# michel-aractingi/soloRL

Measured on AMD Instinct MI355X. Metric: env-steps/s (whole node) Solo12 walk, 4096 envs/GPU, higher is better.
Workload: dtype f32

## Files before the change

solorl_amd/csrc/dynamics.hpp:

```cpp
#pragma once
#include <utility>

#include "../../include/solorl_model_data.h"
#include "spatial.hpp"

namespace solo {

constexpr int MAX_CONTACTS = 8;
constexpr int MAX_LIMITS = 4;
constexpr int LIM_SLOT_ROWS = 2;
constexpr int MAX_ROWS = LIM_SLOT_ROWS + 3 * MAX_CONTACTS;
SD int extra_limits(int nlt) { return nlt > LIM_SLOT_ROWS ? nlt - LIM_SLOT_ROWS : 0; }
SD int contact_cap(int nlt) { return MAX_CONTACTS - extra_limits(nlt); }
constexpr int ROW_CORE = 20;
constexpr int NPRIM = 24;
constexpr double LIMIT_WINDOW = 0.0;
constexpr double DISC_EPS2 = 1e-12;
constexpr double DISC_RIM = 0.1;

#if defined(SOLO_WAVE_TIMING) && !defined(SOLO_HOST_SHIM)
constexpr int SOLO_WT_WAVES = 65536, SOLO_WT_FIELDS = 28;
__device__ unsigned long long solo_wave_times[SOLO_WT_WAVES][SOLO_WT_FIELDS];
__shared__ unsigned long long solo_pt_acc[10];
#define SOLO_PT_DECL() long long pt_last_ = 0
// ... 1231 lines not shown
      }
    }
    mask = team_or16(keep);
  }
  const int nl = __builtin_popcount(lbits);
  if (valid && t >= 4 && ((mask >> (t - 4)) & 1)) {
    const int p = t - 4, nlt = nl, nc = __builtin_popcount(mask);
    const int cidx = __builtin_popcount(mask & ((1 << p) - 1));
    const int sn_ = nlt + cidx, sf_ = nlt + nc + 2 * cidx;
    const T lam0 = pp.warm * C.lamp[p];
    const T Z[3] = {T(0), T(0), T(0)};
    static_for<3>([&](auto dc) {
      constexpr int d = decltype(dc)::value;
      const V3<T> u = d == 0 ? mk(T(0), T(0), T(1)) : (d == 1 ? mk(T(1), T(0), T(0)) : mk(T(0), T(1), T(0)));
      park_row(lds, d == 0 ? sn_ : sf_ + (d - 1), SV<T>{cross(bP, u), u}, Z, Z, bP, bdist + pp.slop, d == 0 ? lam0 : T(0), bfric,
               (d == 0 ? 0 : (sn_ | 128)) | (d << 8));
    });
  }
  if (!lead) return;
  C.R0 = R0;
  C.mask = mask; C.nc = __builtin_popcount(mask); C.nlim_total = nl; C.lsel = lbits;
  C.smask = sbits & mask;
  constexpr solorl_link_data B = RB::MD.links[0];
  static_assert(B.com[0] == 0.0 && B.com[1] == 0.0 && B.com[2] == 0.0, "base COM at its origin");
  RBI<T> Ib; SV<T> pb;
  const SV<T> vb{st.w, st.v};
  SOLO_LINK_TERMS_CE(UI, B, R0, mk(T(0), T(0), T(0)), vb, pp.damping, Ib, pb);
  C.Ibase = to_abi(Ib); C.pbase = pb;
}

template <typename T, int ROBOT, typename CH>
SD void team_sum_base(CH ch, int t) {
  SubCtx<T, ROBOT>& C = ch.get();
  constexpr int NA = (int)(sizeof(ABI<T>) / sizeof(T)), NP = (int)(sizeof(SV<T>) / sizeof(T));
  static_assert(NA == 21 && NP == 6, "ABI / SV are plain arrays of T");
  T* ib = reinterpret_cast<T*>(&C.Ibase); T* pb = reinterpret_cast<T*>(&C.pbase);
  const T* il = reinterpret_cast<const T*>(&C.Ileg[0]); const T* pl = reinterpret_cast<const T*>(&C.pleg[0]);
#pragma unroll
  for (int k = 0; k < 2; k++) {
    const int i = t + 16 * k;
    if (i < NA) ib[i] = ib[i] + ((il[i] + il[NA + i]) + (il[2 * NA + i] + il[3 * NA + i]));
    else if (i < NA + NP) { const int j = i - NA; pb[j] = pb[j] + ((pl[j] + pl[NP + j]) + (pl[2 * NP + j] + pl[3 * NP + j])); }
  }
}

template <typename T, int ROBOT, typename LDS, typename CH>
SNI_SCALAR void phase_base_lead(CH ch, const PhysParams<T> pp, const T* lam_prev, unsigned nstride, const LDS lds) {
  SubCtx<T, ROBOT>& C = ch.get();
  using TRW = TeamRows<T, LDS>;
  constexpr int LN = LDS::LANES;
  const int nlt = C.nlim_total, nc = C.nc;
  const ABI<T> Ib = C.Ibase;
  const SV<T> pb = C.pbase;
  const V3<T> bw = C.ps.w, bv = C.ps.v;
  const Sym6<T> Lam = spd_inverse_block(Ib);
  const SV<T> a0 = mul(Lam, pb) * T(-1);
  const T dt = pp.dt;
  V3<T> vdot = a0.l + cross(bw, bv); vdot.z -= pp.gravity;
  SV<T> ub;
  ub.a = mk(clampv(bw.x + dt * a0.a.x, pp.vmax), clampv(bw.y + dt * a0.a.y, pp.vmax), clampv(bw.z + dt * a0.a.z, pp.vmax));
  ub.l = mk(clampv(bv.x + dt * vdot.x, pp.vmax), clampv(bv.y + dt * vdot.y, pp.vmax), clampv(bv.z + dt * vdot.z, pp.vmax));
  if (nlt + 3 * nc == 0) {
    const T Z[3] = {T(0), T(0), T(0)};
    park_row(lds, 0, zero6<T>(), Z, Z, mk(T(0), T(0), T(0)), T(0), T(0), T(0), 0);
  }
  C.ub = ub;
  T* bc = TRW::bc(lds.lane);
#pragma unroll
  for (int i = 0; i < 6; i++)
#pragma unroll
    for (int j = 0; j < 6; j++) bc[i * 6 + j] = Lam.m[i][j];
  bc[36] = ub.a.x; bc[37] = ub.a.y; bc[38] = ub.a.z; bc[39] = ub.l.x; bc[40] = ub.l.y; bc[41] = ub.l.z;
  bc[54] = a0.a.x; bc[55] = a0.a.y; bc[56] = a0.a.z; bc[57] = a0.l.x; bc[58] = a0.l.y; bc[59] = a0.l.z;
  T* hdr = lds.hdr();
  hdr[0] = T(nlt); hdr[LN] = T(nc);
}

template <typename T, int ROBOT, typename LDS, typename CH>
SD void phase_legrates_team(CH ch, const PhysParams<T> pp, const LDS lds, int t) {
  using RB = Robot<ROBOT>;
  using TRW = TeamRows<T, LDS>;
  constexpr int NJ = RB::NJ;
  T* bc = TRW::bc(lds.lane);
  if (t < RB::NQ) {
    SubCtx<T, ROBOT>& C = ch.get();
    const int L = t / NJ, k = t - L * NJ;
    const SV<T> a0{{bc[54], bc[55], bc[56]}, {bc[57], bc[58], bc[59]}};
    const T qdd = C.LR[L].qdd0[k] - dot(C.LR[L].G[k], a0);
    const T v = clampv(C.ps.qd[t] + pp.dt * qdd, pp.vmax);
    C.qds[t] = v;
    bc[42 + L * 3 + k] = v;
  } else if (NJ < 3 && t < 12) {
    if ((t - RB::NQ) < 4) bc[42 + (t - RB::NQ) * 3 + 2] = T(0);
  }
}

template <typename T, typename LDS> SD void team_counts(const LDS& lds, int& nlt, int& nc, int& ncmax, int& anylim) {
  const T* hdr = lds.hdr();
  nlt = (int)hdr[0]; nc = (int)hdr[LDS::LANES];
  int m = (nc + extra_limits(nlt)) | (nlt << 8);
#pragma unroll
  for (int o = 32; o >= 16; o >>= 1) { int v = __shfl_xor(m, o); m = ((v & 255) > (m & 255) ? (v & 255) : (m & 255)) | ((v | m) & ~255); }
  m = __builtin_amdgcn_readfirstlane(m);
  ncmax = m & 255; anylim = m >> 8;
}

template <typename T, int ROBOT, typename LDS>
SNI_SCALAR void phase_finish_team(const PhysParams<T> pp, const LDS lds, int t) {
  using TRW = TeamRows<T, LDS>;
  const int col = lds.lane;
  int nlt, nc, ncmax, anylim;
  team_counts<T, LDS>(lds, nlt, nc, ncmax, anylim);
  const int nrows = nlt + 3 * nc, rfric = nlt + nc;
  T* const lam = TRW::lam(col);
  const T* bc = TRW::bc(col);
  for (int pos = t; pos < TRW::TR; pos += 16)
    if (TRW::row_of(pos, nlt, nc) < 0) lam[pos * 4] = T(0);
  if (t >= nrows) return;
  Sym6<T> Lam;
#pragma unroll
  for (int i = 0; i < 6; i++)
#pragma unroll
    for (int j = 0; j < 6; j++) Lam.m[i][j] = bc[i * 6 + j];
  const SV<T> ub{{bc[36], bc[37], bc[38]}, {bc[39], bc[40], bc[41]}};
  const int r1 = t + 16;
  const bool two = r1 < nrows;
  T c0[ROW_CORE], c1[ROW_CORE];
  lds.load_core(t, c0);
  const int meta0 = (int)lds.A(t, LDS::A_META);
  const T mu0 = lds.A(t, LDS::A_MU);
  int meta1 = 0; T mu1 = T(1);
  if (two) { lds.load_core(r1, c1); meta1 = (int)lds.A(r1, LDS::A_META); mu1 = lds.A(r1, LDS::A_MU); }
  auto emit = [&](int r, const T (&c)[ROW_CORE], int meta, T mu) __attribute__((always_inline)) {
    const int leg = (meta >> 5) & 3;
    const T* ql = bc + 42 + leg * 3;
    SV<T> W; T rhs, dinv;
    finish_row(c, meta, Lam, ub, ql[0], ql[1], ql[2], pp, W, rhs, dinv);
    const bool fr = r >= rfric;
    const T sB = fr ? mu : T(1);
    const T isB = rcp_fast(sB);
    const T sJ = dinv * isB;
    T o[ROW_CORE];
#pragma unroll
    for (int e = 0; e < 9; e++) o[E_J(e)] = c[e] * sJ;
    o[E_B(0)] = W.a.x * sB; o[E_B(1)] = W.a.y * sB; o[E_B(2)] = W.a.z * sB; o[E_B(3)] = W.l.x * sB; o[E_B(4)] = W.l.y * sB; o[E_B(5)] = W.l.z * sB;
    o[E_B(6)] = c[15] * sB; o[E_B(7)] = c[16] * sB; o[E_B(8)] = c[17] * sB;
    o[E_RHS] = rhs * isB;
    o[E_LEG] = T(leg);
    lds.store_core(r, o);
    lds.A(r, LDS::A_LAM) = (fr && pp.cone()) ? rcp_fast(pp.resid_thr * sJ) : pp.resid_thr * sJ;
    lam[TRW::pos_of(r, nlt, nc) * 4] = c[13];
  };
  emit(t, c0, meta0, mu0);
  if (two) emit(r1, c1, meta1, mu1);
}

template <typename T> SD T half_swap(T x) {
  if constexpr (sizeof(T) == 4) return __int_as_float(__builtin_amdgcn_mov_dpp(__float_as_int(x), 0x140, 0xF, 0xF, true));
  else return __shfl_xor(x, 8, 16);
}

template <typename T> SD T team_red8(T x) {
  if constexpr (sizeof(T) == 4) {
    x += __int_as_float(__builtin_amdgcn_mov_dpp(__float_as_int(x), 0xB1, 0xF, 0xF, true));
    x += __int_as_float(__builtin_amdgcn_mov_dpp(__float_as_int(x), 0x4E, 0xF, 0xF, true));
    x += __int_as_float(__builtin_amdgcn_mov_dpp(__float_as_int(x), 0x141, 0xF, 0xF, true));
  } else {
    x += __shfl_xor(x, 1, 16); x += __shfl_xor(x, 2, 16); x += __shfl_xor(x, 4, 16);
  }
  return x;
}

#ifndef SOLO_SETUP_GROUP_F32
#define SOLO_SETUP_GROUP_F32 5
#endif
#ifndef SOLO_SETUP_GROUP_F64
#define SOLO_SETUP_GROUP_F64 1
#endif
template <typename T, typename LDS, int LIM, int NNS, int NFS, bool EXIT, bool PIPE = true, bool CONE = false>
SNI void pgs_team_variant(int iterations_v, const LDS lds, int t) {
  using TRW = TeamRows<T, LDS>;
  const int itv = __builtin_amdgcn_readfirstlane(iterations_v);
  const int iterations = itv & 0xFFFF;
  const bool warm_on = (itv >> 30) & 1;
  constexpr int LN = LDS::LANES, n = LIM + NNS + NFS;
  constexpr int S_N0 = 1, S_F0 = 1 + MAX_CONTACTS / 2;
  static_assert(n >= 1, "empty sweeps are not instantiated");
  struct Ord { static constexpr int slot(int i) { return i < LIM ? 0 : (i < LIM + NNS ? S_N0 + (i - LIM) : S_F0 + (i - LIM - NNS)); } };
  const int col = lds.lane;
  const int h = t & 7, half = t >> 3;
  constexpr int SZ = (int)sizeof(T);
  constexpr int S_LAM = 4 * SZ;
  const int lam_own = (int)TRW::off_lam + col * SZ + half * S_LAM;
  const int nlt = (int)lds.hdr()[0], nc = (int)lds.hdr()[LN];
  const int eU = h;
  const int legU = h < 6 ? -1 : 0;
  const int eV = 6 + (h + 2) % 3, legV = (h + 2) / 3;
  const int eW = h < 2 ? 7 + h : 8, legW = h < 2 ? 3 : -2;
  constexpr unsigned ROWB = (unsigned)LDS::NCH * LN * 16u;
  auto eoff = [&](int e) -> unsigned { return (unsigned)(e / LDS::PER) * (LN * 16u) + (unsigned)(e % LDS::PER) * SZ + (unsigned)col * 16u; };
  using P2 = T __attribute__((ext_vector_type(2)));
  static_assert(LDS::PER % 2 == 0, "a (J', B~) pair lies inside one 16-byte chunk");
  const unsigned kU = eoff(E_J(eU)), kV = eoff(E_J(eV)), kW = eoff(E_J(eW));
  const unsigned kUB = eoff(E_B(eU)), kVB = eoff(E_B(eV)), kWB = eoff(E_B(eW));
  const unsigned kLEG = eoff(E_LEG), kRHS = eoff(E_RHS);
  auto rd = [&](unsigned rb, unsigned k) -> T { return *reinterpret_cast<const T*>(solo_smem + (rb + k)); };
  auto rd2 = [&](unsigned rb, unsigned k) -> P2 { return *reinterpret_cast<const P2*>(solo_smem + (rb + k)); };
  auto fm = [](auto a, auto b, auto c) { return __builtin_elementwise_fma(a, b, c); };
  T J0[n], J1[n], J2[n], B2[n], X2[n], rh[n], cp[n], lm[n], eo[n], ex[n];
  P2 B01[n], X01[n];
  T th[EXIT ? n : 1];
  T thx[(EXIT && CONE && NFS > 0) ? NFS : 1];
  T lmo[NNS > 0 ? NNS : 1];
  P2 a01 = {T(0), T(0)}; T a2 = T(0);
  int rown[n], roth[n];
  T lego[n], legx[n];
  T ju[n], bu[n], jv[n], bv[n], jw[n], bw[n], xu[n], xv[n], xw[n], rhs_[n];
  constexpr int SETUP_GROUP = sizeof(T) == 4 ? SOLO_SETUP_GROUP_F32 : SOLO_SETUP_GROUP_F64;
  static_for<(n + SETUP_GROUP - 1) / SETUP_GROUP>([&](auto gc) {
    constexpr int g0 = decltype(gc)::value * SETUP_GROUP, gn = (n - g0 < SETUP_GROUP ? n - g0 : SETUP_GROUP);
    static_for<gn>([&](auto jc) {
      constexpr int i = g0 + decltype(jc)::value;
      constexpr int k = Ord::slot(i);
      constexpr bool fr = i >= LIM + NNS;
      rown[i] = TRW::row_of(2 * k + half, nlt, nc);
      if constexpr (fr) roth[i] = rown[i] < 0 ? -1 : rown[i] + 1 - 2 * half;
      else roth[i] = TRW::row_of(2 * k + 1 - half, nlt, nc);
      const int ro = rown[i] < 0 ? 0 : rown[i], rx = roth[i] < 0 ? 0 : roth[i];
      const unsigned bo = __umul24((unsigned)ro, ROWB), bx = __umul24((unsigned)rx, ROWB);
      lego[i] = rd(bo, kLEG);
      if constexpr (!fr) legx[i] = rd(bx, kLEG); else legx[i] = T(0);
      { const P2 u = rd2(bo, kU), v = rd2(bo, kV), w = rd2(bo, kW);
        ju[i] = u.x; bu[i] = u.y; jv[i] = v.x; bv[i] = v.y; jw[i] = w.x; bw[i] = w.y; }
      xu[i] = rd(bx, kUB); xv[i] = rd(bx, kVB); xw[i] = rd(bx, kWB);
      rhs_[i] = rd(bo, kRHS);
      if constexpr (EXIT) th[i] = lds.A(ro, LDS::A_LAM);
      lm[i] = *reinterpret_cast<const T*>(solo_smem + lam_own + 2 * k * S_LAM);
    });
#ifndef SOLO_HOST_SHIM
    asm volatile("" ::: "memory");
    static_for<gn>([&](auto jc) {
      constexpr int i = g0 + decltype(jc)::value;
      asm volatile("" : "+v"(ju[i]), "+v"(bu[i]), "+v"(jv[i]), "+v"(bv[i]), "+v"(jw[i]), "+v"(bw[i]), "+v"(xu[i]), "+v"(xv[i]), "+v"(xw[i]),
                        "+v"(rhs_[i]), "+v"(lm[i]), "+v"(lego[i]));
      (void)legx;
      if constexpr (i < LIM + NNS) asm volatile("" : "+v"(legx[i]));
      (void)th;
      if constexpr (EXIT) asm volatile("" : "+v"(th[i]));
    });
#endif
    static_for<gn>([&](auto jc) {
      constexpr int i = g0 + decltype(jc)::value;
      constexpr bool fr = i >= LIM + NNS;
      const int r_own = rown[i], r_oth = roth[i];
      const int lo = r_own < 0 ? -3 : (int)lego[i], lx = fr ? lo : (r_oth < 0 ? -3 : (int)legx[i]);
      const bool uo = r_own >= 0 && (legU == -1 || legU == lo), vo = legV == lo, wo = legW == lo;
      const bool ux = fr ? uo : (r_oth >= 0 && (legU == -1 || legU == lx)), vx = fr ? vo : legV == lx, wx = fr ? wo : legW == lx;
      J0[i] = uo ? ju[i] : T(0); J1[i] = vo ? jv[i] : T(0); J2[i] = wo ? jw[i] : T(0);
      B01[i] = P2{uo ? bu[i] : T(0), vo ? bv[i] : T(0)}; B2[i] = wo ? bw[i] : T(0);
      X01[i] = P2{ux ? xu[i] : T(0), vx ? xv[i] : T(0)}; X2[i] = wx ? xw[i] : T(0);
      rh[i] = r_own >= 0 ? rhs_[i] * T(-0.125) : T(0);
      if constexpr (CONE && fr) {
        cp[i] = T(0);
        (void)thx;
        if constexpr (EXIT) { if (r_own < 0) th[i] = T(0); thx[i - LIM - NNS] = half_swap(th[i]); }
      } else {
        const T c = team_red8(J0[i] * X01[i].x + J1[i] * X01[i].y + J2[i] * X2[i]);
        cp[i] = half ? c : T(0);
      }
      if constexpr (i >= LIM && i < LIM + NNS) lmo[i - LIM] = T(0);
    });
    if (warm_on) {
      static_for<gn>([&](auto jc) {
        constexpr int i = g0 + decltype(jc)::value;
        const T lx_ = half_swap(lm[i]);
        if constexpr (i >= LIM && i < LIM + NNS) lmo[i - LIM] = lx_;
        a01 = fm(X01[i], P2{lx_, lx_}, fm(B01[i], P2{lm[i], lm[i]}, a01)); a2 = fm(X2[i], lx_, fm(B2[i], lm[i], a2));
      });
    }
  });
  static_for<n>([&](auto ic) {
    constexpr int i = decltype(ic)::value, p = (i + n - 1) % n;
    if constexpr (PIPE) {
      eo[i] = team_red8(J0[i] * B01[p].x + J1[i] * B01[p].y + J2[i] * B2[p]);
      ex[i] = team_red8(J0[i] * X01[p].x + J1[i] * X01[p].y + J2[i] * X2[p]);
    } else { eo[i] = T(0); ex[i] = T(0); (void)p; }
  });
  auto jdot = [&](int, T j0, T j1, T j2, T r8) -> T { return team_red8(fm(j0, a01.x, fm(j1, a01.y, fm(j2, a2, r8)))); };
  T dpre = jdot(0, J0[0], J1[0], J2[0], rh[0]);
  T delp = T(0), delxp = T(0);
  T* const hdr = lds.hdr();
#define SOLO_PGS_WRITE_BACK() do { \
    if (h == 0) { \
      static_for<n>([&](auto ic_) { \
        constexpr int i_ = decltype(ic_)::value; \
        *reinterpret_cast<T*>(solo_smem + lam_own + 2 * Ord::slot(i_) * S_LAM) = lm[i_]; \
      }); \
    } \
    if (half == 0) { \
      if (h < 6) hdr[(2 + h) * LN] = a01.x; else lds.y()[(h - 6) * LN] = a01.x; \
      lds.y()[(h + 2) * LN] = a01.y; \
      if (h < 2) lds.y()[(10 + h) * LN] = a2; \
    } } while (0)
  bool fin = false;
#if defined(SOLO_WAVE_TIMING) && defined(SOLO_DEAD_STATS)
  unsigned long long fr_tot = 0, fr_dead = 0;
#endif
  int it_done = 0; (void)it_done;
#pragma unroll 1
  for (int it = 0; it < iterations; it++) {
#if defined(SOLO_WAVE_TIMING) && defined(SOLO_SWEEP_STATS)
    it_done = it + 1;
#endif
    bool viol = false;
    static_for<n>([&](auto ic) {
      constexpr int i = decltype(ic)::value, in = (i + 1) % n;
      constexpr bool fric = i >= LIM + NNS;
      T dnext = T(0), d;
      if constexpr (PIPE) {
        dnext = jdot(in, J0[in], J1[in], J2[in], rh[in]);
        d = fm(ex[i], delxp, fm(eo[i], delp, dpre));
      } else d = jdot(i, J0[i], J1[i], J2[i], rh[i]);
      T hi = T(0);
      if constexpr (fric) {
        constexpr int c = i - LIM - NNS;
        if constexpr (sizeof(T) == 4) hi = __int_as_float(__builtin_amdgcn_mov_dpp(__float_as_int(lm[LIM + (c >> 1)]), 0x150 + 8 * (c & 1), 0xF, 0xF, true));
        else hi = (half == (c & 1)) ? lm[LIM + (c >> 1)] : lmo[c >> 1];
      }
      auto clampb = [&](T x) -> T {
        if constexpr (!fric) return x > T(0) ? x : T(0);
        else if constexpr (sizeof(T) == 4) return __builtin_amdgcn_fmed3f(x, -hi, hi);
        else return x < -hi ? -hi : (x > hi ? hi : x);
      };
#if defined(SOLO_WAVE_TIMING) && defined(SOLO_DEAD_STATS)
      if constexpr (fric) { fr_tot++; if (!__any(hi != T(0) || lm[i] != T(0))) fr_dead++; }
#endif
      T sp = lm[i] - d;
      T sv;
      if constexpr (CONE && fric) {
        const T spx = half_swap(sp);
        const T s2 = fm(sp, sp, fm(spx, spx, T(1e-30)));
        T sc;
        if constexpr (sizeof(T) == 4) {
#ifndef SOLO_HOST_SHIM
          sc = __builtin_amdgcn_fmed3f(hi * __builtin_amdgcn_rsqf(s2), 0.0f, 1.0f);
#else
          sc = hi / sqrt(s2); sc = sc < T(1) ? sc : T(1);
#endif
        } else { sc = hi / sqrt(s2); sc = sc < T(1) ? sc : T(1); }
        sv = sp * sc;
      } else {
        const T dfirst = clampb(sp) - lm[i];
        sp = fm(-cp[i], half_swap(dfirst), sp);
        sv = clampb(sp);
      }
      const T del = sv - lm[i];
      lm[i] = sv;
      const T delx = half_swap(del);
      if constexpr (EXIT) {
        if constexpr (CONE && fric) viol = viol || (fabs(fm(delx, thx[i - LIM - NNS], del * th[i])) > T(1));
        else viol = viol || (fabs(del) > th[i]);
      }
      if constexpr (sizeof(T) != 4 && i >= LIM && i < LIM + NNS) lmo[i - LIM] += delx;
      a01 = fm(X01[i], P2{delx, delx}, fm(B01[i], P2{del, del}, a01));
      a2 = fm(X2[i], delx, fm(B2[i], del, a2));
      dpre = dnext; delp = del; delxp = delx;
    });
    if constexpr (EXIT) {
      const bool quiet = team_or16(viol ? 1 : 0) == 0;
      const bool nw = quiet && !fin;
      if (__any(nw)) {
        if (nw) SOLO_PGS_WRITE_BACK();
        fin = fin || quiet;
        if (__all(fin)) break;
      }
    }
  }
  if constexpr (EXIT) { if (!fin) SOLO_PGS_WRITE_BACK(); }
  else SOLO_PGS_WRITE_BACK();
#if defined(SOLO_WAVE_TIMING) && defined(SOLO_SWEEP_STATS)
  if (threadIdx.x == 0 && blockIdx.x < SOLO_WT_WAVES) { solo_wave_times[blockIdx.x][26] += (unsigned long long)it_done; solo_wave_times[blockIdx.x][27] += 1ull; }
#endif
#if defined(SOLO_WAVE_TIMING) && defined(SOLO_DEAD_STATS)
  if (threadIdx.x == 0 && blockIdx.x < SOLO_WT_WAVES) { solo_wave_times[blockIdx.x][26] += fr_tot; solo_wave_times[blockIdx.x][27] += fr_dead; }
#endif
#undef SOLO_PGS_WRITE_BACK
}

template <typename T, int ROBOT, typename LDS>
SD void phase_pgs_team(int iterations_, bool warm_on, bool early_exit, bool pipe, bool cone, const LDS lds, int t) {
  const int iterations = (iterations_ & 0xFFFF) | (warm_on ? 1 << 30 : 0);
  constexpr int LN = LDS::LANES;
  int nlt, nc, ncmax, anylim;
  team_counts<T, LDS>(lds, nlt, nc, ncmax, anylim);
#if defined(SOLO_WAVE_TIMING)
  if (threadIdx.x == 0 && blockIdx.x < SOLO_WT_WAVES) {
    solo_wave_times[blockIdx.x][4] += (unsigned long long)(ncmax + (ncmax + 1) / 2 + (anylim ? 1 : 0));
    if ((unsigned long long)ncmax > solo_wave_times[blockIdx.x][5]) solo_wave_times[blockIdx.x][5] = (unsigned long long)ncmax;
  }
#endif
#ifndef SOLO_NO_SETPRIO
  if (ncmax >= 7) __builtin_amdgcn_s_setprio(3);
  else if (ncmax >= 5) __builtin_amdgcn_s_setprio(2);
  else if (ncmax >= 3) __builtin_amdgcn_s_setprio(1);
  else __builtin_amdgcn_s_setprio(0);
#endif
#define SOLO_SWEEP_C(N_, F_, C_) do { if (early_exit) { if (anylim) pgs_team_variant<T, LDS, 1, N_, F_, true, true, C_>(iterations, lds, t); \
                                                        else pgs_team_variant<T, LDS, 0, N_, F_, true, true, C_>(iterations, lds, t); } \
                                      else if (pipe) { if (anylim) pgs_team_variant<T, LDS, 1, N_, F_, false, true, C_>(iterations, lds, t); \
                                                       else pgs_team_variant<T, LDS, 0, N_, F_, false, true, C_>(iterations, lds, t); } \
                                      else { if (anylim) pgs_team_variant<T, LDS, 1, N_, F_, false, false, C_>(iterations, lds, t); \
                                             else pgs_team_variant<T, LDS, 0, N_, F_, false, false, C_>(iterations, lds, t); } } while (0)
#define SOLO_SWEEP_L(N_, F_) do { if (cone) SOLO_SWEEP_C(N_, F_, true); else SOLO_SWEEP_C(N_, F_, false); } while (0)
  switch (ncmax) {
    case 0:
      if (anylim) { if (early_exit) pgs_team_variant<T, LDS, 1, 0, 0, true>(iterations, lds, t); else pgs_team_variant<T, LDS, 1, 0, 0, false>(iterations, lds, t); }
      else {
        const int h = t & 7;
        T* const hdr = lds.hdr();
        if ((t >> 3) == 0) {
          if (h < 6) hdr[(2 + h) * LN] = T(0); else lds.y()[(h - 6) * LN] = T(0);
          lds.y()[(h + 2) * LN] = T(0);
          if (h < 2) lds.y()[(10 + h) * LN] = T(0);
        }
      }
      break;
    case 1: SOLO_SWEEP_L(1, 1); break;
    case 2: SOLO_SWEEP_L(1, 2); break;
    case 3: SOLO_SWEEP_L(2, 3); break;
    case 4: SOLO_SWEEP_L(2, 4); break;
    case 5: SOLO_SWEEP_L(3, 5); break;
    case 6: SOLO_SWEEP_L(3, 6); break;
    case 7: SOLO_SWEEP_L(4, 7); break;
    default: SOLO_SWEEP_L(4, 8); break;
  }
#undef SOLO_SWEEP_L
#undef SOLO_SWEEP_C
}

template <typename T, int ROBOT, typename LDS, typename CH>
SNI_SCALAR void phase_integrate_team(CH ch, const PhysParams<T> pp, T* lam_prev, unsigned nstride, const LDS lds, int t, bool valid,
                              bool lead) {
  using RB = Robot<ROBOT>;
  using TRW = TeamRows<T, LDS>;
  constexpr int NJ = RB::NJ, LN = LDS::LANES;
  if (!valid) return;
  SubCtx<T, ROBOT>& C = ch.get();
  const T dt = pp.dt;
  const int mask = C.mask;
  const int nlt = C.nlim_total;
  const T* hdr = lds.hdr();
  const SV<T> w{{hdr[2 * LN], hdr[3 * LN], hdr[4 * LN]}, {hdr[5 * LN], hdr[6 * LN], hdr[7 * LN]}};
  const int tj = t < RB::NQ ? t : 0;
  const int L = tj / NJ, k = tj - L * NJ;
  const T qds = C.qds[tj], yk = lds.y()[(L * 3 + k) * LN], qj = C.ps.q[tj];
  const SV<T> Gk = C.LR[L].G[k];
  const SV<T> ub = C.ub;
  const V3<T> pos = C.ps.pos;
  const T x = C.ps.qx, yq = C.ps.qy, z = C.ps.qz, ww = C.ps.qw;
  const T* lam = TRW::lam(lds.lane);
  const int npos0 = TRW::NPOS0 + extra_limits(nlt);
  T lv[(NPRIM + 15) / 16];
#pragma unroll
  for (int i = 0; i < (NPRIM + 15) / 16; i++) {
    const int p = t + 16 * i;
    const int pp_ = p < NPRIM ? p : 0;
    lv[i] = lam[(npos0 + __builtin_popcount(mask & ((1 << pp_) - 1))) * 4];
    lv[i] = (p < NPRIM && ((mask >> pp_) & 1)) ? lv[i] : T(0);
  }
  const T nvj = clampv(qds + yk - dot(Gk, w), pp.vmax);
  const V3<T> nw = mk(clampv(ub.a.x + w.a.x, pp.vmax), clampv(ub.a.y + w.a.y, pp.vmax), clampv(ub.a.z + w.a.z, pp.vmax));
  const V3<T> nv = mk(clampv(ub.l.x + w.l.x, pp.vmax), clampv(ub.l.y + w.l.y, pp.vmax), clampv(ub.l.z + w.l.z, pp.vmax));
#pragma unroll
  for (int i = 0; i < (NPRIM + 15) / 16; i++) { const int p = t + 16 * i; if (p < NPRIM) C.lamp[p] = lv[i]; }
  if (t < RB::NQ) { C.ps.qd[t] = nvj; C.ps.q[t] = qj + dt * nvj; }
  if (lead) {
    C.ps.w = nw; C.ps.v = nv;
    C.ps.pos = fma3(nv, dt, pos);
    T wn2 = dot(nw, nw), wn = sqrt_fast(wn2), sc, s_, cw;
    sincos_t(T(0.5) * wn * dt, s_, cw);
    if (wn < T(1e-3)) sc = T(0.5) * dt - dt * dt * dt * T(1.0 / 48.0) * wn2; else sc = s_ * rcp_fast(wn);
    T ax = nw.x * sc, ay = nw.y * sc, az = nw.z * sc;
    T nx = cw * x + ax * ww + ay * z - az * yq;
    T ny = cw * yq - ax * z + ay * ww + az * x;
    T nz = cw * z + ax * yq - ay * x + az * ww;
    T nq = cw * ww - ax * x - ay * yq - az * z;
    T inv = rsqrt_fast(nx * nx + ny * ny + nz * nz + nq * nq);
    C.ps.qx = nx * inv; C.ps.qy = ny * inv; C.ps.qz = nz * inv; C.ps.qw = nq * inv;
  }
}

template <typename T, int ROBOT, typename LDS> struct TeamCtx {
  using type = CtxLds<T, ROBOT, TeamRows<T, LDS>::off_ctx>;
  static constexpr size_t bytes = TeamRows<T, LDS>::off_ctx + 4 * sizeof(SubCtx<T, ROBOT>);
};

template <typename T, int ROBOT, typename LDS>
SD int substep_team(const PhysParams<T> pp, T* lam_prev, unsigned nstride, const LDS& lds, int t, bool lead, bool valid) {
  constexpr int LN = LDS::LANES;
  using TRW = TeamRows<T, LDS>;
  using CH = typename TeamCtx<T, ROBOT, LDS>::type;
  const CH ch{lds.lane};
  SOLO_PT_DECL();
  SOLO_PT_BEGIN();
  if (valid && t < Robot<ROBOT>::NQ) {
    SubCtx<T, ROBOT>& C = ch.get();
    T sn, cs;
    sincos_t(C.ps.q[t], sn, cs);
    C.sn[t] = sn; C.cs[t] = cs;
  }
  SOLO_PT(0);
  const bool ui = pp.urdf_inertia();
  if (ui) phase_front_team<T, ROBOT, LDS, CH, true>(ch, pp, lds, t, valid, lead);
  else phase_front_team<T, ROBOT, LDS, CH, false>(ch, pp, lds, t, valid, lead);
  SOLO_PT(1);
#if SOLO_LEG_QUAD
  if (valid) {
    if (ui) phase_leg_rt<T, ROBOT, LDS, CH, true>(ch, pp, lam_prev, nstride, lds, t >> 2, t & 3);
    else phase_leg_rt<T, ROBOT, LDS, CH, false>(ch, pp, lam_prev, nstride, lds, t >> 2, t & 3);
  }
#else
  if (valid && t < 4) {
    if (ui) phase_leg_rt<T, ROBOT, LDS, CH, true>(ch, pp, lam_prev, nstride, lds, t, 0);
    else phase_leg_rt<T, ROBOT, LDS, CH, false>(ch, pp, lam_prev, nstride, lds, t, 0);
  }
#endif
  SOLO_PT(2);
  if (valid) team_sum_base<T, ROBOT, CH>(ch, t);
  SOLO_PT(3);
  if (lead) phase_base_lead<T, ROBOT, LDS, CH>(ch, pp, lam_prev, nstride, lds);
  else if (!valid && t == 0) {
    lds.hdr()[0] = T(0); lds.hdr()[LN] = T(0);
  }
  SOLO_PT(4);
  if (valid) phase_legrates_team<T, ROBOT, LDS, CH>(ch, pp, lds, t);
  SOLO_PT(5);
  phase_finish_team<T, ROBOT, LDS>(pp, lds, t);
  SOLO_PT(6);
  phase_pgs_team<T, ROBOT, LDS>(pp.iterations, pp.warm != T(0), pp.resid_thr >= T(0), pp.pgs_pipe(), pp.cone(), lds, t);
  SOLO_PT(7);
  phase_integrate_team<T, ROBOT, LDS, CH>(ch, pp, lam_prev, nstride, lds, t, valid, lead);
  SOLO_PT(8);
  return lead ? (ch.get().mask | strip_feet_bits(ch.get().smask)) : 0;
}
#endif

template <typename T, int ROBOT, typename LDS>
SD int substep(SubCtx<T, ROBOT>& C, const PhysParams<T> pp, T* lam_prev, unsigned nstride, const LDS& lds) {
  using CH = CtxPriv<T, ROBOT>;
  const CH ch{&C};
  if (pp.urdf_inertia()) {
    phase_detect<T, ROBOT, CH, true>(ch, pp);
    phase_leg<T, ROBOT, 0, LDS, CH, true>(ch, pp, lam_prev, nstride, lds);
    phase_leg<T, ROBOT, 1, LDS, CH, true>(ch, pp, lam_prev, nstride, lds);
    phase_leg<T, ROBOT, 2, LDS, CH, true>(ch, pp, lam_prev, nstride, lds);
    phase_leg<T, ROBOT, 3, LDS, CH, true>(ch, pp, lam_prev, nstride, lds);
  } else {
    phase_detect<T, ROBOT, CH, false>(ch, pp);
    phase_leg<T, ROBOT, 0, LDS, CH, false>(ch, pp, lam_prev, nstride, lds);
    phase_leg<T, ROBOT, 1, LDS, CH, false>(ch, pp, lam_prev, nstride, lds);
    phase_leg<T, ROBOT, 2, LDS, CH, false>(ch, pp, lam_prev, nstride, lds);
    phase_leg<T, ROBOT, 3, LDS, CH, false>(ch, pp, lam_prev, nstride, lds);
  }
  phase_base<T, ROBOT, LDS, CH>(ch, pp, lam_prev, nstride, lds);
  if (pp.cone()) phase_pgs<T, ROBOT, LDS, CH, true>(ch, pp.iterations, pp.resid_thr, lds);
  else phase_pgs<T, ROBOT, LDS, CH>(ch, pp.iterations, pp.resid_thr, lds);
  phase_integrate<T, ROBOT, LDS, CH>(ch, pp, lam_prev, nstride, lds);
  return C.mask | strip_feet_bits(C.smask);
}

}
```

solorl_amd/devcode.py:

```python
import os
import re
import subprocess
import tempfile

LLVM = os.environ.get("ROCM_LLVM_BIN", "/opt/rocm/lib/llvm/bin")


MAGIC = b"__CLANG_OFFLOAD_BUNDLE__"


def _code_objects(lib_path, workdir):
    fat = os.path.join(workdir, "fat.bin")
    subprocess.check_call([os.path.join(LLVM, "llvm-objcopy"), "--dump-section", ".hip_fatbin=" + fat, lib_path, os.path.join(workdir, "x.so")])
    blob = open(fat, "rb").read()
    starts = [m.start() for m in re.finditer(re.escape(MAGIC), blob)]
    out = []
    for k, a in enumerate(starts):
        part = os.path.join(workdir, "fat%d.bin" % k)
        open(part, "wb").write(blob[a:starts[k + 1] if k + 1 < len(starts) else len(blob)])
        co = os.path.join(workdir, "dev%d.co" % k)
        subprocess.check_call([os.path.join(LLVM, "clang-offload-bundler"), "--unbundle", "--type=o", "--input=" + part,
                               "--targets=hipv4-amdgcn-amd-amdhsa--gfx950", "--output=" + co])
        if os.path.getsize(co) > 0:
            out.append(co)
    return out


def disassemble(lib_path):
    out, seen = [], {}
    with tempfile.TemporaryDirectory() as d:
        for co in _code_objects(lib_path, d):
            for line in subprocess.check_output([os.path.join(LLVM, "llvm-objdump"), "-d", co], text=True).splitlines():
                m = re.match(r"^([0-9a-f]+) <([^>]+)>:", line)
                if m:
                    k = seen.get(m.group(2), 0)
                    seen[m.group(2)] = k + 1
                    if k:
                        line = "%s <%s.dup%d>:" % (m.group(1), m.group(2), k)
                out.append(line)
    return "\n".join(out)


def kernel_static_lds(lib_path):
    with tempfile.TemporaryDirectory() as d:
        notes = "\n".join(subprocess.check_output([os.path.join(LLVM, "llvm-readelf"), "--notes", co], text=True) for co in _code_objects(lib_path, d))
    out, size = {}, None
    for line in notes.splitlines():
        m = re.search(r"\.group_segment_fixed_size:\s*(\d+)", line)
        if m:
            size = int(m.group(1))
        m = re.search(r"^\s*\.name:\s*(\S+)", line)
        if m and size is not None:
            out[m.group(1)] = size
            size = None
    return out


def kernel_resources(lib_path):
    with tempfile.TemporaryDirectory() as d:
        notes = "\n".join(subprocess.check_output([os.path.join(LLVM, "llvm-readelf"), "--notes", co], text=True) for co in _code_objects(lib_path, d))
    out, cur, col = {}, None, None
    for line in notes.splitlines():
        m = re.match(r"^(\s*-?\s*)\.([a-z_]+):\s*(\S*)\s*$", line)
        if not m:
            continue
        if m.group(1).strip() == "-" and m.group(2) == "agpr_count":
            cur, col = {}, len(m.group(1))
        if cur is None or len(m.group(1)) != col:
            continue
        if m.group(2) == "name":
            out[m.group(3)] = cur
        elif m.group(3).isdigit():
            cur[m.group(2)] = int(m.group(3))
    return out


def function_stats(lib_path):
    out, cur = {}, None
    for line in disassemble(lib_path).splitlines():
        m = re.match(r"^[0-9a-f]+ <([^>]+)>:", line)
        if m:
            cur = out.setdefault(m.group(1), dict(insts=0, scratch=0, flat=0, **{"global": 0})) if ".dup" not in m.group(1) else None
            continue
        if cur is None or "\t" not in line:
            continue
        op = line.split("\t")[1].strip().split(" ")[0] if len(line.split("\t")) > 1 else ""
        if not op:
            continue
        cur["insts"] += 1
        if op.startswith("scratch_"): cur["scratch"] += 1
        elif op.startswith("flat_"): cur["flat"] += 1
        elif op.startswith("global_"): cur["global"] += 1
    return out


def loop_stats(lib_path, name_filter):
    funcs, cur = {}, None
    for line in disassemble(lib_path).splitlines():
        m = re.match(r"^[0-9a-f]+ <([^>]+)>:", line)
        if m:
            cur = funcs.setdefault(m.group(1), [])
            continue
        if cur is not None and "\t" in line:
            cur.append(line)
    out = {}
    off_re = re.compile(r"//\s*([0-9A-Fa-f]+):")
    for name, lines in funcs.items():
        if name_filter not in name or not lines or ".dup" in name:
            continue
        base = int(off_re.search(lines[0]).group(1), 16)
        rows = []
        for l in lines:
            mo = off_re.search(l)
            if mo:
                rows.append((int(mo.group(1), 16) - base, l.split("\t")[1].strip() if len(l.split("\t")) > 1 else ""))
        lo = hi = None
        for off, op in rows:
            if op.startswith(("s_cbranch", "s_branch")):
                mt = re.search(r"<[^>]*\+0x([0-9a-f]+)>", op)
                if mt and int(mt.group(1), 16) < off and off - int(mt.group(1), 16) > 200:
                    if lo is None or off - int(mt.group(1), 16) > hi - lo:
                        lo, hi = int(mt.group(1), 16), off
        inl = [op for off, op in rows if lo is not None and lo <= off <= hi]
        out[name] = dict(insts=len(rows), scratch=sum(op.startswith("scratch_") for _, op in rows), loop=(lo, hi),
                         scratch_in_loop=sum(op.startswith("scratch_") for op in inl), valu_in_loop=sum(op.startswith("v_") for op in inl),
                         lds_in_loop=sum(op.startswith("ds_") for op in inl), lds_reads_in_loop=sum(op.startswith("ds_read") for op in inl),
                         vmem_in_loop=sum(op.startswith(("global_", "flat_", "buffer_")) for op in inl))
    return out


if __name__ == "__main__":
    import sys
    from .build import LIB
    for name, s in sorted(function_stats(sys.argv[1] if len(sys.argv) > 1 else LIB).items()):
        if s["insts"] > 100:
            print("%-120s insts %6d scratch %4d flat %4d global %4d" % (name[:120], s["insts"], s["scratch"], s["flat"], s["global"]))
```

Baseline: 23.61 million.

## Hand-schedule PGS sweep with sched barriers and ballot-based early exit

```diff
diff --git a/solorl_amd/csrc/dynamics.hpp b/solorl_amd/csrc/dynamics.hpp
--- a/solorl_amd/csrc/dynamics.hpp
+++ b/solorl_amd/csrc/dynamics.hpp
@@ -1557,81 +1557,157 @@
       lds.y()[(h + 2) * LN] = a01.y; \
       if (h < 2) lds.y()[(10 + h) * LN] = a2; \
     } } while (0)
-  bool fin = false;
+  unsigned long long finm = 0; (void)finm;
+  if constexpr (EXIT) finm = ~__builtin_amdgcn_ballot_w64(true);
 #if defined(SOLO_WAVE_TIMING) && defined(SOLO_DEAD_STATS)
   unsigned long long fr_tot = 0, fr_dead = 0;
 #endif
   int it_done = 0; (void)it_done;
 #pragma unroll 1
-  for (int it = 0; it < iterations; it++) {
+  for (int it = iterations; it > 0; it--) {
 #if defined(SOLO_WAVE_TIMING) && defined(SOLO_SWEEP_STATS)
-    it_done = it + 1;
-#endif
-    bool viol = false;
+    it_done++;
+#endif
+    unsigned long long violm = 0; (void)violm;
+    T vmax = T(0); (void)vmax;
     static_for<n>([&](auto ic) {
       constexpr int i = decltype(ic)::value, in = (i + 1) % n;
       constexpr bool fric = i >= LIM + NNS;
-      T dnext = T(0), d;
-      if constexpr (PIPE) {
-        dnext = jdot(in, J0[in], J1[in], J2[in], rh[in]);
+      T dnext = T(0), d = T(0), sv, del, delx, tx = T(0);
+      (void)d; (void)tx;
+#if defined(SOLO_WAVE_TIMING) && defined(SOLO_DEAD_STATS)
+      constexpr bool SCHED = false, SCHEDN = false;
+#else
+      constexpr bool SCHED = PIPE && CONE && fric && sizeof(T) == 4;
+      constexpr bool SCHEDN = PIPE && !fric && sizeof(T) == 4;
+#endif
+#define SOLO_SB() __builtin_amdgcn_sched_barrier(0)
+#define SOLO_DPP_ADD(x_, ctrl_) ((x_) + __int_as_float(__builtin_amdgcn_mov_dpp(__float_as_int(x_), ctrl_, 0xF, 0xF, true)))
+      if constexpr (SCHED) {
+        constexpr int c = i - LIM - NNS;
+        SOLO_SB();
         d = fm(ex[i], delxp, fm(eo[i], delp, dpre));
-      } else d = jdot(i, J0[i], J1[i], J2[i], rh[i]);
-      T hi = T(0);
-      if constexpr (fric) {
-        constexpr int c = i - LIM - NNS;
-        if constexpr (sizeof(T) == 4) hi = __int_as_float(__builtin_amdgcn_mov_dpp(__float_as_int(lm[LIM + (c >> 1)]), 0x150 + 8 * (c & 1), 0xF, 0xF, true));
-        else hi = (half == (c & 1)) ? lm[LIM + (c >> 1)] : lmo[c >> 1];
+        const T sp = lm[i] - d;
+        SOLO_SB();
+        dnext = fm(J0[in], a01.x, fm(J1[in], a01.y, fm(J2[in], a2, rh[in])));
+        SOLO_SB();
+        const T spx = half_swap(sp);
+        T s2 = fm(spx, spx, T(1e-30));
+        SOLO_SB();
+        dnext = SOLO_DPP_ADD(dnext, 0xB1);
+        SOLO_SB();
+        s2 = fm(sp, sp, s2);
+        const T rs = __builtin_amdgcn_rsqf(s2);
+        SOLO_SB();
+        dnext = SOLO_DPP_ADD(dnext, 0x4E);
+        SOLO_SB();
+        const T hi = __int_as_float(__builtin_amdgcn_mov_dpp(__float_as_int(lm[LIM + (c >> 1)]), 0x150 + 8 * (c & 1), 0xF, 0xF, true));
+        const T sc = __builtin_amdgcn_fmed3f(hi * rs, 0.0f, 1.0f);
+        del = fm(sp, sc, -lm[i]);
+        SOLO_SB();
+        dnext = SOLO_DPP_ADD(dnext, 0x141);
+        sv = sp * sc;
+        if constexpr (EXIT) tx = del * th[i];
+        SOLO_SB();
+        delx = half_swap(del);
+        SOLO_SB();
+      } else if constexpr (SCHEDN) {
+        SOLO_SB();
+        d = fm(ex[i], delxp, fm(eo[i], delp, dpre));
+        T sp = lm[i] - d;
+        const T dfirst = (sp > T(0) ? sp : T(0)) - lm[i];
+        SOLO_SB();
+        dnext = fm(J0[in], a01.x, fm(J1[in], a01.y, fm(J2[in], a2, rh[in])));
+        SOLO_SB();
+        sp = fm(-cp[i], half_swap(dfirst), sp);
+        SOLO_SB();
+        dnext = SOLO_DPP_ADD(dnext, 0xB1);
+        SOLO_SB();
+        sv = sp > T(0) ? sp : T(0);
+        del = sv - lm[i];
+        SOLO_SB();
+        dnext = SOLO_DPP_ADD(dnext, 0x4E);
+        a01 = fm(B01[i], P2{del, del}, a01);
+        SOLO_SB();
+        delx = half_swap(del);
+        SOLO_SB();
+        dnext = SOLO_DPP_ADD(dnext, 0x141);
+        SOLO_SB();
+      } else {
+        if constexpr (PIPE) {
+          dnext = jdot(in, J0[in], J1[in], J2[in], rh[in]);
+          d = fm(ex[i], delxp, fm(eo[i], delp, dpre));
+        } else d = jdot(i, J0[i], J1[i], J2[i], rh[i]);
+        T hi = T(0);
+        if constexpr (fric) {
+          constexpr int c = i - LIM - NNS;
+          if constexpr (sizeof(T) == 4) hi = __int_as_float(__builtin_amdgcn_mov_dpp(__float_as_int(lm[LIM + (c >> 1)]), 0x150 + 8 * (c & 1), 0xF, 0xF, true));
+          else hi = (half == (c & 1)) ? lm[LIM + (c >> 1)] : lmo[c >> 1];
+        }
+        auto clampb = [&](T x) -> T {
+          if constexpr (!fric) return x > T(0) ? x : T(0);
+          else if constexpr (sizeof(T) == 4) return __builtin_amdgcn_fmed3f(x, -hi, hi);
+          else return x < -hi ? -hi : (x > hi ? hi : x);
+        };
+#if defined(SOLO_WAVE_TIMING) && defined(SOLO_DEAD_STATS)
+        if constexpr (fric) { fr_tot++; if (!__any(hi != T(0) || lm[i] != T(0))) fr_dead++; }
+#endif
+        T sp = lm[i] - d;
+        if constexpr (CONE && fric) {
+          const T spx = half_swap(sp);
+          const T s2 = fm(sp, sp, fm(spx, spx, T(1e-30)));
+          T sc;
+          if constexpr (sizeof(T) == 4) {
+#ifndef SOLO_HOST_SHIM
+            sc = __builtin_amdgcn_fmed3f(hi * __builtin_amdgcn_rsqf(s2), 0.0f, 1.0f);
+#else
+            sc = hi / sqrt(s2); sc = sc < T(1) ? sc : T(1);
+#endif
+          } else { sc = hi / sqrt(s2); sc = sc < T(1) ? sc : T(1); }
+          del = fm(sp, sc, -lm[i]);
+          if constexpr (sizeof(T) == 4) asm("" : "+v"(sp) : "v"(del));
+          sv = sp * sc;
+        } else {
+          const T dfirst = clampb(sp) - lm[i];
+          sp = fm(-cp[i], half_swap(dfirst), sp);
+          sv = clampb(sp);
+          del = sv - lm[i];
+        }
+        delx = half_swap(del);
+        if constexpr (EXIT && CONE && fric) tx = del * th[i];
       }
-      auto clampb = [&](T x) -> T {
-        if constexpr (!fric) return x > T(0) ? x : T(0);
-        else if constexpr (sizeof(T) == 4) return __builtin_amdgcn_fmed3f(x, -hi, hi);
-        else return x < -hi ? -hi : (x > hi ? hi : x);
-      };
-#if defined(SOLO_WAVE_TIMING) && defined(SOLO_DEAD_STATS)
-      if constexpr (fric) { fr_tot++; if (!__any(hi != T(0) || lm[i] != T(0))) fr_dead++; }
-#endif
-      T sp = lm[i] - d;
-      T sv;
-      if constexpr (CONE && fric) {
-        const T spx = half_swap(sp);
-        const T s2 = fm(sp, sp, fm(spx, spx, T(1e-30)));
-        T sc;
-        if constexpr (sizeof(T) == 4) {
-#ifndef SOLO_HOST_SHIM
-          sc = __builtin_amdgcn_fmed3f(hi * __builtin_amdgcn_rsqf(s2), 0.0f, 1.0f);
-#else
-          sc = hi / sqrt(s2); sc = sc < T(1) ? sc : T(1);
-#endif
-        } else { sc = hi / sqrt(s2); sc = sc < T(1) ? sc : T(1); }
-        sv = sp * sc;
-      } else {
-        const T dfirst = clampb(sp) - lm[i];
-        sp = fm(-cp[i], half_swap(dfirst), sp);
-        sv = clampb(sp);
-      }
-      const T del = sv - lm[i];
       lm[i] = sv;
-      const T delx = half_swap(del);
       if constexpr (EXIT) {
-        if constexpr (CONE && fric) viol = viol || (fabs(fm(delx, thx[i - LIM - NNS], del * th[i])) > T(1));
-        else viol = viol || (fabs(del) > th[i]);
+        if constexpr (CONE && fric) {
+          const T x = fabs(fm(delx, thx[i - LIM - NNS], tx));
+          if constexpr (sizeof(T) == 4) vmax = __builtin_fmaxf(vmax, x); else vmax = __builtin_fmax(vmax, x);
+        } else violm |= __builtin_amdgcn_ballot_w64(fabs(del) > th[i]);
       }
       if constexpr (sizeof(T) != 4 && i >= LIM && i < LIM + NNS) lmo[i - LIM] += delx;
-      a01 = fm(X01[i], P2{delx, delx}, fm(B01[i], P2{del, del}, a01));
+      if constexpr (SCHEDN) a01 = fm(X01[i], P2{delx, delx}, a01);
+      else a01 = fm(X01[i], P2{delx, delx}, fm(B01[i], P2{del, del}, a01));
       a2 = fm(X2[i], delx, fm(B2[i], del, a2));
       dpre = dnext; delp = del; delxp = delx;
-    });
+#undef SOLO_DPP_ADD
+#undef SOLO_SB
+    });
+    if constexpr (PIPE && sizeof(T) == 4) asm volatile("" :: "v"(dpre));
     if constexpr (EXIT) {
-      const bool quiet = team_or16(viol ? 1 : 0) == 0;
-      const bool nw = quiet && !fin;
-      if (__any(nw)) {
+      if constexpr (CONE && NFS > 0) violm |= __builtin_amdgcn_ballot_w64(vmax > T(1));
+      const unsigned long long vm = violm | finm;
+      if (((vm - 0x0001000100010001ull) & ~vm & 0x8000800080008000ull) != 0) {
+        const int row = __builtin_amdgcn_mbcnt_hi(~0u, __builtin_amdgcn_mbcnt_lo(~0u, 0u)) & 48;
+        const bool nw = ((unsigned)(vm >> row) & 0xFFFFu) == 0;
         if (nw) SOLO_PGS_WRITE_BACK();
-        fin = fin || quiet;
-        if (__all(fin)) break;
+        finm |= __builtin_amdgcn_ballot_w64(nw);
+        if (finm == ~0ull) it = 1;
       }
     }
   }
-  if constexpr (EXIT) { if (!fin) SOLO_PGS_WRITE_BACK(); }
+  if constexpr (EXIT) {
+    const int ln = __builtin_amdgcn_mbcnt_hi(~0u, __builtin_amdgcn_mbcnt_lo(~0u, 0u));
+    if (!((finm >> ln) & 1)) SOLO_PGS_WRITE_BACK();
+  }
   else SOLO_PGS_WRITE_BACK();
 #if defined(SOLO_WAVE_TIMING) && defined(SOLO_SWEEP_STATS)
   if (threadIdx.x == 0 && blockIdx.x < SOLO_WT_WAVES) { solo_wave_times[blockIdx.x][26] += (unsigned long long)it_done; solo_wave_times[blockIdx.x][27] += 1ull; }
diff --git a/solorl_amd/devcode.py b/solorl_amd/devcode.py
--- a/solorl_amd/devcode.py
+++ b/solorl_amd/devcode.py
@@ -123,6 +123,7 @@
                         lo, hi = int(mt.group(1), 16), off
         inl = [op for off, op in rows if lo is not None and lo <= off <= hi]
         out[name] = dict(insts=len(rows), scratch=sum(op.startswith("scratch_") for _, op in rows), loop=(lo, hi),
+                         insts_in_loop=len(inl), s_nop_in_loop=sum(op.startswith("s_nop") for op in inl),
                          scratch_in_loop=sum(op.startswith("scratch_") for op in inl), valu_in_loop=sum(op.startswith("v_") for op in inl),
                          lds_in_loop=sum(op.startswith("ds_") for op in inl), lds_reads_in_loop=sum(op.startswith("ds_read") for op in inl),
                          vmem_in_loop=sum(op.startswith(("global_", "flat_", "buffer_")) for op in inl))
```

Result: faster. 25.82 million (median of 6 runs) (+9.4%).
